# AhmedKishki/AMP-SPARC-SpatialModulation

Hardware: AMD Instinct MI355X
Metric: detected symbol-vectors/sec, VAMP Nt=256 Nr=512 16-QAM; SER match vs ref (higher is better)
Workload: dtype bf16x3; 1 GPU; cfg4: VAMP Nt=256 Nr=512 Na=8 16QAM batch=4096 iterations<=20 EbN0=8.0 dB, one channel per batch; global_batch=4096, parallelism=epoch-shard x1 (independent epochs, one all-reduce of the error counters)

## Files before the change

amp-sparc-spatialmodulation_amd/csrc/amp_persist.h:

```cpp
#pragma once

#include <cfloat>

#include "amp_common.h"

namespace amp {

constexpr int PRING = 4;

typedef float f32x4 __attribute__((ext_vector_type(4)));
typedef unsigned u32x4 __attribute__((ext_vector_type(4)));

__device__ __forceinline__ f32x4 mfma16x16x4(float a, float b, f32x4 c) {
    return __builtin_amdgcn_mfma_f32_16x16x4f32(a, b, c, 0, 0, 0);
}

template <int NT, int G>
__device__ __forceinline__ void gemm16(const float* sA, int lda, const float* __restrict__ wq, int ct0,
                                       f32x4 (&acc)[NT]) {
    constexpr int R = G < PRING ? G : PRING;
    const int lane = threadIdx.x & 63;
#pragma unroll
    for (int t = 0; t < NT; ++t) acc[t] = f32x4{0.f, 0.f, 0.f, 0.f};
    const int ct0u = __builtin_amdgcn_readfirstlane(ct0);
// ... 87 lines not shown
    u32x4 q[6];
#pragma unroll
    for (int h = 0; h < 4; ++h) {
        unsigned a0, a1, a2, b0, b1, b2;
        split3x2(re[2 * h], re[2 * h + 1], a0, a1, a2);
        split3x2(im[2 * h], im[2 * h + 1], b0, b1, b2);
        q[0][h] = a0; q[1][h] = a1; q[2][h] = a2; q[3][h] = b0; q[4][h] = b1; q[5][h] = b2;
    }
    const int c = pl_col(pl_opaque(row), j0, pl_mask(ldx));
#pragma unroll
    for (int f = 0; f < 6; ++f) *reinterpret_cast<u32x4*>(sP + (f * 16 + row) * ldx + c) = q[f];
}

__device__ __forceinline__ float dpp_swap_pair(float v) {
    return __int_as_float(__builtin_amdgcn_update_dpp(0, __float_as_int(v), 0xB1, 0xF, 0xF, false));
}

__device__ __forceinline__ void x3_store_acc(unsigned short* sP, int ldx, int o, const float (&vr)[4],
                                             const float (&vi)[4]) {
    const int lane = pl_opaque((int)threadIdx.x) & 63;
    const bool odd = (lane & 1) != 0;
    float gr[2], gi[2];
#pragma unroll
    for (int h = 0; h < 2; ++h) {
        gr[h] = dpp_swap_pair(odd ? vr[h] : vr[2 + h]);
        gi[h] = dpp_swap_pair(odd ? vi[h] : vi[2 + h]);
    }
    const int row0 = 4 * (lane >> 4) + (odd ? 2 : 0);
    const int m = pl_mask(ldx);
    const int pl = 16 * ldx;
#pragma unroll
    for (int h = 0; h < 2; ++h) {
        unsigned short* p = sP + (row0 + h) * ldx + pl_col(row0 + h, o & ~1, m);
        const float mr = odd ? vr[2 + h] : vr[h], mi = odd ? vi[2 + h] : vi[h];
        unsigned q[6];
        split3x2(odd ? gr[h] : mr, odd ? mr : gr[h], q[0], q[1], q[2]);
        split3x2(odd ? gi[h] : mi, odd ? mi : gi[h], q[3], q[4], q[5]);
#pragma unroll
        for (int f = 0; f < 6; ++f) *reinterpret_cast<unsigned*>(p + f * pl) = q[f];
    }
}

__device__ __forceinline__ void split3(float x, unsigned& p0, unsigned& p1, unsigned& p2) {
    unsigned q0, q1, q2;
    split3x2(x, 0.0f, q0, q1, q2);
    p0 = q0 & 0xffffu; p1 = q1 & 0xffffu; p2 = q2 & 0xffffu;
}

__device__ __forceinline__ bf16x8 as_bf16x8(u32x4 v) { return __builtin_bit_cast(bf16x8, v); }

constexpr int x3_ring_depth(int G, int R) { return G < R ? G : R; }
template <int NT, int RR>
struct X3Ring {
    u32x4 v[RR][NT][6];
};

template <int G>
__device__ __forceinline__ __amdgpu_buffer_rsrc_t x3_wrsrc(const void* wq, int ct0) {
    const int ct0u = __builtin_amdgcn_readfirstlane(ct0);
    return __builtin_amdgcn_make_buffer_rsrc((char*)const_cast<void*>(wq) + (size_t)ct0u * G * 6 * 1024, (short)0,
                                             0x7ffffff0, 0x00020000);
}

template <int NT, int G, int RR, int T0 = 0, int T1 = NT>
__device__ __forceinline__ void x3_ring_load(X3Ring<NT, RR>& ring, int d, __amdgpu_buffer_rsrc_t wr, int g) {
    const int vo = (threadIdx.x & 63) * 16;
#pragma unroll
    for (int t = T0; t < T1; ++t)
#pragma unroll
        for (int f = 0; f < 6; ++f)
            ring.v[d][t][f] = __builtin_amdgcn_raw_buffer_load_b128(wr, vo, ((t * G + g) * 6 + f) * 1024, 0);
}

template <int NT, int G, int R = 1, int T0 = 0, int T1 = NT>
__device__ __forceinline__ void x3_ring_fill(X3Ring<NT, x3_ring_depth(G, R)>& ring, const void* __restrict__ wq, int ct0) {
    const __amdgpu_buffer_rsrc_t wr = x3_wrsrc<G>(wq, ct0);
#pragma unroll
    for (int d = 0; d < x3_ring_depth(G, R); ++d) x3_ring_load<NT, G, x3_ring_depth(G, R), T0, T1>(ring, d, wr, d);
}

struct X3NoHook {
    __device__ __forceinline__ void operator()(int) const {}
};
template <int NT, int G, int R = 1, bool PIN = false, bool HL = false, bool NEXT = false, class Hook = X3NoHook>
__device__ __forceinline__ void gemm_x3_ring(const unsigned short* sP, int ldx, const void* __restrict__ wq, int ct0,
                                             X3Ring<NT, x3_ring_depth(G, R)>& ring, f32x4 (&cr)[NT], f32x4 (&ci)[NT],
                                             const void* __restrict__ wq_next = nullptr, Hook&& hook = Hook()) {
    constexpr int RR = x3_ring_depth(G, R);
    static_assert(!NEXT || G % RR == 0, "the next operator's group j lands in slot j % RR");
    constexpr int NL = HL ? NT : 1;
    const int lane = threadIdx.x & 63;
    f32x4 lr[NL], li[NL];
#pragma unroll
    for (int t = 0; t < NT; ++t) { cr[t] = f32x4{0.f, 0.f, 0.f, 0.f}; ci[t] = f32x4{0.f, 0.f, 0.f, 0.f}; }
#pragma unroll
    for (int t = 0; t < NL; ++t) { lr[t] = f32x4{0.f, 0.f, 0.f, 0.f}; li[t] = f32x4{0.f, 0.f, 0.f, 0.f}; }
    const __amdgpu_buffer_rsrc_t wr = x3_wrsrc<G>(wq, ct0);
    const int ln = pl_opaque(lane);
    const int sw = (ln & 15) & pl_mask(ldx);
    const unsigned short* ap = sP + (ln & 15) * ldx + 8 * ((ln >> 4) ^ (sw & 3));
    const int s32 = 32 * (sw >> 2);
    const u32x4 sgn = {0x80008000u, 0x80008000u, 0x80008000u, 0x80008000u};
    u32x4 an[6];
    if constexpr (!PIN) {
#pragma unroll
        for (int f = 0; f < 6; ++f) an[f] = *reinterpret_cast<const u32x4*>(ap + s32 + f * 16 * ldx);
    }
#pragma unroll
    for (int g = 0; g < G; ++g) {
        const int d = g % RR;
        u32x4 a[6], na[3];
        if constexpr (PIN) {
#pragma unroll
            for (int f = 0; f < 6; ++f) a[f] = *reinterpret_cast<const u32x4*>(ap + ((32 * g) ^ s32) + f * 16 * ldx);
        } else {
#pragma unroll
            for (int f = 0; f < 6; ++f) a[f] = an[f];
            if (g + 1 < G) {
#pragma unroll
                for (int f = 0; f < 6; ++f)
                    an[f] = *reinterpret_cast<const u32x4*>(ap + ((32 * (g + 1)) ^ s32) + f * 16 * ldx);
            }
        }
#pragma unroll
        for (int f = 0; f < 3; ++f) na[f] = a[3 + f] ^ sgn;
#pragma unroll
        for (int t = 0; t < NT; ++t) {
            const u32x4* w = ring.v[d][t];
            f32x4 gr = cr[t], gi = ci[t];
            f32x4 sr = HL ? lr[HL ? t : 0] : gr, si = HL ? li[HL ? t : 0] : gi;
#define AMP_MF(acc, x, y) acc = __builtin_amdgcn_mfma_f32_16x16x32_bf16(as_bf16x8(x), as_bf16x8(y), acc, 0, 0, 0)
            AMP_MF(sr, a[0], w[2]);  AMP_MF(si, a[0], w[5]);
            AMP_MF(sr, a[1], w[1]);  AMP_MF(si, a[1], w[4]);
            AMP_MF(sr, a[2], w[0]);  AMP_MF(si, a[2], w[3]);
            AMP_MF(sr, na[0], w[5]); AMP_MF(si, a[3], w[2]);
            AMP_MF(sr, na[1], w[4]); AMP_MF(si, a[4], w[1]);
            AMP_MF(sr, na[2], w[3]); AMP_MF(si, a[5], w[0]);
            AMP_MF(sr, a[0], w[1]);  AMP_MF(si, a[0], w[4]);
            AMP_MF(sr, a[1], w[0]);  AMP_MF(si, a[1], w[3]);
            AMP_MF(sr, na[0], w[4]); AMP_MF(si, a[3], w[1]);
            AMP_MF(sr, na[1], w[3]); AMP_MF(si, a[4], w[0]);
            if constexpr (HL) {
                lr[HL ? t : 0] = sr; li[HL ? t : 0] = si;
            } else {
                gr = sr; gi = si;
            }
            AMP_MF(gr, a[0], w[0]);  AMP_MF(gi, a[0], w[3]);
            AMP_MF(gr, na[0], w[3]); AMP_MF(gi, a[3], w[0]);
#undef AMP_MF
            cr[t] = gr; ci[t] = gi;
        }
        if constexpr (PIN) __builtin_amdgcn_sched_barrier(0);
        hook(g);
        if (g + RR < G) {
            x3_ring_load<NT, G>(ring, d, wr, g + RR);
        } else if constexpr (NEXT) {
            x3_ring_load<NT, G>(ring, d, x3_wrsrc<G>(wq_next, ct0), g + RR - G);
        }
        __builtin_amdgcn_sched_barrier(0);
    }
    if constexpr (HL) {
#pragma unroll
        for (int t = 0; t < NT; ++t) { cr[t] += lr[HL ? t : 0]; ci[t] += li[HL ? t : 0]; }
    }
}

template <int NT, int G, int R = 1, bool PIN = false, bool HL = false>
__device__ __forceinline__ void gemm_x3(const unsigned short* sP, int ldx, const void* __restrict__ wq, int ct0,
                                        f32x4 (&cr)[NT], f32x4 (&ci)[NT]) {
    X3Ring<NT, x3_ring_depth(G, R)> ring;
    x3_ring_fill<NT, G, R>(ring, wq, ct0);
    gemm_x3_ring<NT, G, R, PIN, HL>(sP, ldx, wq, ct0, ring, cr, ci);
}

typedef _Float16 f16x8 __attribute__((ext_vector_type(8)));
typedef _Float16 f16x2_t __attribute__((ext_vector_type(2)));
constexpr int H2_EX = 14;
constexpr int YH2_EX = 10;

__device__ __forceinline__ int h2_row_exp(float m) {
    if (!(m > 0.f) || !__builtin_isfinite(m)) return 0;
    return 14 - __builtin_amdgcn_frexp_expf(m);
}

__device__ __forceinline__ void split2x2(float x, float y, unsigned& p0, unsigned& p1) {
    const f32x2_t v = {x, y};
    const f16x2_t h0 = __builtin_convertvector(v, f16x2_t);
    const f32x2_t b = __builtin_convertvector(h0, f32x2_t);
    f32x2_t r = v - b;
    r.x = __builtin_isfinite(b.x) ? r.x : 0.0f;
    r.y = __builtin_isfinite(b.y) ? r.y : 0.0f;
    const f16x2_t h1 = __builtin_convertvector(r, f16x2_t);
    p0 = __builtin_bit_cast(unsigned, h0);
    p1 = __builtin_bit_cast(unsigned, h1);
}

__device__ __forceinline__ void split2(float x, int e, unsigned& p0, unsigned& p1) {
    unsigned q0, q1;
    split2x2(__builtin_amdgcn_ldexpf(x, e), 0.0f, q0, q1);
    p0 = q0 & 0xffffu; p1 = q1 & 0xffffu;
}

__device__ __forceinline__ void h2_store8(unsigned short* sP, int ldx, int row, int j0, const float (&re)[8],
                                          const float (&im)[8]) {
    u32x4 q[4];
#pragma unroll
    for (int h = 0; h < 4; ++h) {
        unsigned a0, a1, b0, b1;
        split2x2(re[2 * h], re[2 * h + 1], a0, a1);
        split2x2(im[2 * h], im[2 * h + 1], b0, b1);
        q[0][h] = a0; q[1][h] = a1; q[2][h] = b0; q[3][h] = b1;
    }
    const int c = pl_col(pl_opaque(row), j0, pl_mask(ldx));
#pragma unroll
    for (int f = 0; f < 4; ++f) *reinterpret_cast<u32x4*>(sP + (f * 16 + row) * ldx + c) = q[f];
}

__device__ __forceinline__ void h2_store_acc(unsigned short* sP, int ldx, int o, const float (&vr)[4],
                                             const float (&vi)[4]) {
    const int lane = pl_opaque((int)threadIdx.x) & 63;
    const bool odd = (lane & 1) != 0;
    float gr[2], gi[2];
#pragma unroll
    for (int h = 0; h < 2; ++h) {
        gr[h] = dpp_swap_pair(odd ? vr[h] : vr[2 + h]);
        gi[h] = dpp_swap_pair(odd ? vi[h] : vi[2 + h]);
    }
    const int row0 = 4 * (lane >> 4) + (odd ? 2 : 0);
    const int m = pl_mask(ldx);
    const int pl = 16 * ldx;
#pragma unroll
    for (int h = 0; h < 2; ++h) {
        unsigned short* p = sP + (row0 + h) * ldx + pl_col(row0 + h, o & ~1, m);
        const float mr = odd ? vr[2 + h] : vr[h], mi = odd ? vi[2 + h] : vi[h];
        unsigned q[4];
        split2x2(odd ? gr[h] : mr, odd ? mr : gr[h], q[0], q[1]);
        split2x2(odd ? gi[h] : mi, odd ? mi : gi[h], q[2], q[3]);
#pragma unroll
        for (int f = 0; f < 4; ++f) *reinterpret_cast<unsigned*>(p + f * pl) = q[f];
    }
}
// ... 346 lines not shown
```

amp-sparc-spatialmodulation_amd/csrc/amp_vamp.h:

```cpp
#pragma once

#include "amp_decide.h"
#include "amp_denoise.h"
#include "amp_gemm.h"
#include "amp_host.h"

namespace amp {

constexpr int RWG = 1024;
constexpr int PBAR_EPOCH = 64;
constexpr int PBAR_WORDS = PBAR_EPOCH + 256;

struct VampK {
    int B, N, n, k, L, M;
    int Bmean;
    int kap0, ncp0, kap1, ncp1, kap2, ncp2, bn2;
    int nblk2, max_iter;
    double noise_var, sparsity;
    const float* Wt0;
    const float* Wt1;
    const float* Wt2;
    const float* s;
    float* s2;
    float* ytil;
    float* w;
    float* r;
    float* xm;
    float* var0;
    float* var1;
    float* secmax;
    float* secabs;
    Partial* parts;
    VampIter* iters;
    amp_status* status;
    int nwg;
    int E, wpe;
    const float* Wq1;
    const float* Wq2;
    Partial* pparts;
    double* pxch;
    unsigned* pbar;
    unsigned gen;
    int ytil_in_kernel;
    const float* Wq0;
    const float* y;
    int dec_on, ibits, Na, Lin;
    const float2* xtrue;
    const long long* sym;
    const long long* idx;
    DecWG* dwg;
    unsigned char* host_rec;
    int fold_in;
    amp_counts* counts;
    unsigned long long* trace;
    int x3;
    const void* Wx1;
    const void* Wx2;
    XState* xs;
    float* dump;
    long long wch;
    int sch;
    int wg_off, nwg_x, row_off;
    float* q0;
    int q0_store, q0_load;
    Const c;
};

struct VampWs {
    float *Wt0, *Wt1, *Wt2, *s2, *ytil, *w, *var1;
    float *secmax, *secabs;
    Partial* parts;
    VampIter* iters;
    float *Wq0, *Wq1, *Wq2;
    float *Wx1, *Wx2;
    Partial* pparts;
    double* pxch;
    unsigned* pbar;
    DecWG* dwg;
    XState* xs;
    float* q0;
    size_t bytes;
};

static void vamp_geometry(const amp_dims* d, int k, VampK& P) {
    P.Na = d->Na; P.Lin = d->Lin;
    P.B = d->B; P.N = d->N; P.n = d->n; P.k = k; P.L = d->L; P.M = d->M;
    P.kap0 = round_up(2 * d->n, GBK); P.ncp0 = round_up(2 * k, 128);
    P.kap1 = round_up(2 * d->N, GBK); P.ncp1 = round_up(2 * k, 128);
    P.bn2 = section_bn(d);
    P.kap2 = round_up(2 * k, GBK); P.ncp2 = round_up(2 * d->N, P.bn2);
    P.nblk2 = cdiv(d->B, GBM) * (P.ncp2 / P.bn2);
}

static VampWs vamp_carve(const amp_dims* d, int k, int max_iter, void* base, int chans = 1) {
    VampK P;
    vamp_geometry(d, k, P);
    Carve cv(base);
    VampWs w;
    w.Wt0 = cv.take<float>((size_t)P.ncp0 * P.kap0);
    w.Wt1 = cv.take<float>((size_t)P.ncp1 * P.kap1);
    w.Wt2 = cv.take<float>((size_t)P.ncp2 * P.kap2);
    w.s2 = cv.take<float>((size_t)k);
    w.ytil = cv.take<float>((size_t)d->B * 2 * k);
    w.w = cv.take<float>((size_t)d->B * 2 * k);
    w.var1 = cv.take<float>((size_t)d->B * d->N);
    w.secmax = cv.take<float>((size_t)d->B * d->L);
    w.secabs = cv.take<float>((size_t)d->B * d->L);
    w.parts = cv.take<Partial>((size_t)max_iter * P.nblk2);
    w.iters = cv.take<VampIter>((size_t)max_iter + 1);
    const int nwg = cdiv(d->B, 16);
    w.Wq0 = cv.take<float>((size_t)2 * k * 2 * d->n * chans);
    w.Wq1 = cv.take<float>((size_t)2 * k * 2 * d->N);
    w.Wq2 = cv.take<float>((size_t)2 * d->N * 2 * k);
    w.Wx1 = cv.take<float>((size_t)3 * k * d->N * chans);
    w.Wx2 = cv.take<float>((size_t)3 * k * d->N * chans);
    w.pxch = cv.take<double>((size_t)max_iter * nwg * 4);
    w.pbar = cv.take<unsigned>(PBAR_WORDS);
    w.pparts = cv.take<Partial>((size_t)max_iter * nwg);
    w.dwg = cv.take<DecWG>((size_t)2 * nwg);
    w.xs = cv.take<XState>(1);
    w.q0 = cv.take<float>((size_t)2 * k);
    w.bytes = cv.off;
    return w;
}

__device__ __forceinline__ float* var_buf(const VampK& P, int t) { return (t & 1) ? P.var1 : P.var0; }

struct S2Lane {
    float v[4];
};
__device__ inline S2Lane s2_lane(const VampK& P, const float* s) {
    S2Lane a;
    const int lane = threadIdx.x & 63;
#pragma unroll
    for (int j = 0; j < 4; ++j) {
        const int i = lane + 64 * j;
        const float x = s[min(i, P.k - 1)];
        a.v[j] = i < P.k ? x * x : 0.f;
    }
    return a;
}

__device__ inline void vamp_lmmse_scalars(const VampK& P, bool first, double s2t64, float s2t, float* lds, VampIter& it,
                                          const S2Lane* sl = nullptr) {
    const float vr = first ? (float)(P.noise_var / s2t64) : (1.0f / s2t) * (float)P.noise_var;
    (void)lds;
    double ss = 0.0;
    if (sl) {
        const int lane = threadIdx.x & 63;
#pragma unroll
        for (int j = 0; j < 4; ++j)
            if (lane + 64 * j < P.k) ss += (double)(1.0f / (sl->v[j] + vr));
    } else {
        for (int i = threadIdx.x & 63; i < P.k; i += 64) ss += (double)(1.0f / (P.s[i] * P.s[i] + vr));
    }
    ss = group_sum(ss, 64);
    const float varL = (float)(ss / (double)P.k) * (float)P.noise_var;
    const double eta = (double)P.k / (double)P.N;
    float xtv, s2t32;
    if (first) {
        xtv = (float)eta * varL + (float)((1.0 - eta) * s2t64);
        s2t32 = (float)s2t64;
    } else {
        xtv = (float)eta * varL + (float)(1.0 - eta) * s2t;
        s2t32 = s2t;
    }
    const float alpha = clampf_t(xtv / s2t32, AMP_VAR_RATIO_MIN, 1.0f - AMP_VAR_RATIO_MIN);
    const float sigma2 = clampf_t((alpha / (1.0f - alpha)) * s2t32, AMP_VAR_MIN, AMP_VAR_MAX);
    it.vr = vr;
    it.alpha = alpha;
    it.inv1ma = 1.0f / (1.0f - alpha);
    it.sigma2 = sigma2;
    it.inv_sigma2 = 1.0f / sigma2;
    it.s2t = s2t32;
}

__device__ inline VampIter vamp_first_iter(const VampK& P, float* lds, const S2Lane* sl = nullptr) {
    VampIter it;
    it.stopped = 0; it.T = 0; it.fixed = 0; it.fixed_all = 0; it.G = 0.0;
    it.pad1[0] = it.pad1[1] = it.pad1[2] = 0.f;
    it.dxdr_prev = 0.f;
    it.ns_prev = 1.f;
    const double p = P.sparsity;
    vamp_lmmse_scalars(P, true, p * p * (1 - p) + (1 - p) * (1 - p) * p, 0.f, lds, it, sl);
    return it;
}

__device__ inline VampIter vamp_advance(const VampK& P, const VampIter& cur, const PartAcc& pa, int fixed, int t,
                                        float* lds, const S2Lane* sl = nullptr) {
    VampIter nx;
    nx.stopped = 0; nx.T = 0; nx.fixed = fixed; nx.fixed_all = (fixed < 0) ? 1 : 0; nx.G = pa.maxabs;
    nx.pad1[0] = nx.pad1[1] = nx.pad1[2] = 0.f;
    if (pa.notclose == 0) {
        nx = cur;
        nx.stopped = 1;
        nx.T = t + 1;
        nx.fixed = fixed;
    } else {
        const float mean = (float)(pa.sumvar / ((double)P.Bmean * (double)P.N));
        const float dxdr = clampf_t(mean / cur.sigma2, AMP_VAR_RATIO_MIN, 1.0f - AMP_VAR_RATIO_MIN);
        const float ns = 1.0f / (1.0f - dxdr);
        const float s2t = clampf_t((cur.sigma2 * dxdr) * ns, AMP_VAR_MIN, AMP_VAR_MAX);
        nx.dxdr_prev = dxdr;
        nx.ns_prev = ns;
        vamp_lmmse_scalars(P, false, 0.0, s2t, lds, nx, sl);
    }
    return nx;
}

__device__ inline amp_status vamp_make_status(const VampK& P, const VampIter& cur, const VampIter& nx, int fixed) {
    amp_status s;
    s.T = nx.stopped ? nx.T : P.max_iter;
    s.nan_state = fixed != 0 ? 1 : 0;
    s.stopped = nx.stopped;
    s.gemm = P.x3 + 1;
    s.last_scalar[0] = cur.s2t; s.last_scalar[1] = cur.alpha; s.last_scalar[2] = cur.sigma2;
    s.last_scalar[3] = nx.stopped ? cur.dxdr_prev : nx.dxdr_prev;
    return s;
}

struct PDenoisePolicy {
    const float* r;
    float* x;
    float* vnew;
    const float* vprev;
    float* sm;
    float* sa;
    int ldr, M, lspr, N;
    float inv;
    __device__ __forceinline__ void load(int sec, int m, float& rr, float& ri, float& it) const {
        const int row = sec >> lspr, sj = sec & ((1 << lspr) - 1);
        const float2 v = *reinterpret_cast<const float2*>(r + row * ldr + 2 * (sj * M + m));
        rr = v.x; ri = v.y; it = inv;
    }
    __device__ __forceinline__ void store(int sec, int m, float xr, float xi, float var, PartAcc& pa) const {
        const int row = sec >> lspr, sj = sec & ((1 << lspr) - 1);
        *reinterpret_cast<float2*>(x + row * ldr + 2 * (sj * M + m)) = make_float2(xr, xi);
        const int vo = row * N + sj * M + m;
        vnew[vo] = var;
        pa.sumvar += (double)var;
        pa.notclose += torch_close(var, vprev[vo]) ? 0u : 1u;
    }
    __device__ __forceinline__ void section(int sec, float smax, float sabs) const {
        sm[sec] = smax;
        sa[sec] = sabs;
    }
    __device__ __forceinline__ void load_r(int sec, int m, float& rr, float& ri) const {
        const int row = sec >> lspr, sj = sec & ((1 << lspr) - 1);
        const float2 v = *reinterpret_cast<const float2*>(r + row * ldr + 2 * (sj * M + m));
        rr = v.x; ri = v.y;
    }
    __device__ __forceinline__ float load_prev(int sec, int m) const {
        const int row = sec >> lspr, sj = sec & ((1 << lspr) - 1);
        return vprev[row * N + sj * M + m];
    }
    __device__ __forceinline__ void store_xv(int sec, int m, float xr, float xi, float var) const {
        const int row = sec >> lspr, sj = sec & ((1 << lspr) - 1);
        *reinterpret_cast<float2*>(x + row * ldr + 2 * (sj * M + m)) = make_float2(xr, xi);
        vnew[row * N + sj * M + m] = var;
    }
    __device__ __forceinline__ void account(float var, float vp, PartAcc& pa) const {
        pa.sumvar += (double)var;
        pa.notclose += torch_close(var, vp) ? 0u : 1u;
    }
    float* dbg = nullptr;
};
__device__ __forceinline__ void den_debug(const PDenoisePolicy& p, int sec, int m, float ze, float vs) {
    if (p.dbg) {
        const int row = sec >> p.lspr, sj = sec & ((1 << p.lspr) - 1);
        p.dbg[row * 2 * p.N + sj * p.M + m] = ze;
        p.dbg[row * 2 * p.N + p.N + sj * p.M + m] = vs;
    }
}

constexpr int PBM = 16;

bool vamp_persist_eligible(const amp_dims* d, int k, int ncu, int epochs = 1, int gemm = AMP_GEMM_AUTO);
int vamp_persist_max_epochs(const amp_dims* d, int k, int ncu, int gemm = AMP_GEMM_AUTO);
int vamp_persist_wg_per_cu(const amp_dims* d, int k, int gemm);
int vamp_gemm_select(const amp_dims* d, int k, int gemm);
bool vamp_persist_x3_fits(int N, int k, int L);
bool vamp_persist_ytil_in_kernel(const VampK& P);
bool vamp_persist_ytil_h2(const VampK& P);
int vamp_persist_launch(const VampK& P, const Const64& c64, const DecConst& dc, hipStream_t st, int ncu);
int device_cu_count();
float* debug_dump_ptr();
bool gemm_f32_requested();
bool persist_wg2();

}
```

amp-sparc-spatialmodulation_amd/csrc/amp_vamp_persist_kernel.h:

```cpp
#pragma once

#include <stdlib.h>

#include <type_traits>

#include "amp_decide_fused.h"
#include "amp_persist.h"
#include "amp_vamp.h"

namespace amp {

constexpr int AMP_TRACE_STRIDE = 10;
#ifndef AMP_OCC2_PK
#define AMP_OCC2_PK 0
#endif
#ifndef AMP_KK4_DU
#define AMP_KK4_DU 4
#endif
#ifndef AMP_X3_W8_PIN
#define AMP_X3_W8_PIN 0
#endif
#ifndef AMP_X3_W8_RING
#define AMP_X3_W8_RING 1
#endif
#ifndef AMP_X3_W8_PKGRID
#define AMP_X3_W8_PKGRID 1
#endif
#ifndef AMP_X3_W8_DENFAST
#define AMP_X3_W8_DENFAST 1
#endif
#ifndef AMP_DECIDE_NARROW
#define AMP_DECIDE_NARROW 1
#endif
#ifndef AMP_X3_DU
#define AMP_X3_DU 2
#endif

struct PLayout {
    int lda, ldr;
    int offA, offR, offX, offV0, offV1, offSM, offSA, offScr, total;
};

__host__ __device__ inline int x3_ldx(int N) { return pl_ldx(N); }
__host__ __device__ inline int x3_plane_floats(int N) { return 6 * 16 * x3_ldx(N) / 2; }

__host__ __device__ inline PLayout playout(int N, int k, int L, bool x3 = false) {
    PLayout y;
    y.lda = (2 * N > 2 * k ? 2 * N : 2 * k) + 4;
    y.ldr = 2 * N + (x3 ? 8 : 4);
    int o = 0;
    y.offA = o; o += (x3 && x3_plane_floats(N) > PBM * y.lda) ? x3_plane_floats(N) : PBM * y.lda;
    y.offR = o; o += PBM * y.ldr;
    y.offX = o; o += PBM * y.ldr;
    y.offV0 = o; o += PBM * N;
    y.offV1 = o; o += PBM * N;
    y.offSM = o; o += PBM * L;
    y.offSA = o; o += PBM * L;
    o = (o + 3) & ~3;
    y.offScr = o; o += 1024;
    y.total = o;
    return y;
}

constexpr int KARG_DC_OFF = karg_second_offset<VampK, DecConst>();

template <int NT, int KK, int NWV, int DU, bool X3, int OCC = 1, bool H2 = false, bool I8 = false>
__global__ __launch_bounds__(64 * NWV, OCC * NWV / 4) void vamp_persist(VampK P_arg, DecConst dc_arg) {
    (void)P_arg;
    (void)dc_arg;
    unsigned long long kbase = karg_base();
    const VampK* Pp = karg_at<VampK>(kbase, 0);
    const DecConst* Dp = karg_at<DecConst>(kbase, KARG_DC_OFF);
#define P (*Pp)
#define dc (*Dp)
    static_assert(!X3 || ((NWV == 4 || (NWV == 8 && !H2 && OCC == 1)) && NT % 2 == 0),
                  "X3: four waves (eight for the bf16x3 two-waves-per-SIMD form), whole complex tiles");
    static_assert(!(H2 && I8) && (!I8 || X3), "I8: a split-precision form of its own");
    constexpr int PKDEN = ((OCC * NWV / 4 == 1) || AMP_OCC2_PK) ? PK_ALL
                          : (NWV == 8 && KK == 16 && AMP_X3_W8_PKGRID) ? PK_GRID : PK_NONE;
    constexpr bool DENFAST = NWV == 8 && OCC == 1 && PKDEN == PK_GRID && AMP_X3_W8_DENFAST;
    constexpr int PWG = 64 * NWV;
    constexpr int NC = X3 ? NT / 2 : 1;
    constexpr int G3 = NT * NWV / 4;
    constexpr int X3R = (NWV == 8) ? AMP_X3_W8_RING : 1;
    constexpr bool X3PIN = NWV == 8 && AMP_X3_W8_PIN;
    constexpr bool X3PF = X3 && !H2 && !I8;
    constexpr int PFT = (NC + 1) / 2;
#define c64 (static_cast<const Const64&>(*Dp))
    extern __shared__ __attribute__((aligned(16))) float lds[];
    __shared__ int s_flag;
    __shared__ double s_d[PWG / 64][4];
    __shared__ float s_hmax[PWG / 64][PBM];
    __shared__ int s_hexp[PBM];
    const PLayout Y = playout(P.N, P.k, P.L, X3);
    float* sA = lds + Y.offA;
    float* sR = lds + Y.offR;
    float* sX = lds + Y.offX;
    float* sM = lds + Y.offSM;
    float* sS = lds + Y.offSA;
    float* scr = lds + Y.offScr;
    const int tid = threadIdx.x, lane = tid & 63, wave = tid >> 6;
    const int wg = blockIdx.x, nwg = gridDim.x;
    const int wgx = wg + P.wg_off, nwx = P.nwg_x;
    const int ep = wgx / P.wpe, wl = wgx - ep * P.wpe, wg0 = ep * P.wpe;
    const int lrow0 = wl * PBM;
    const int row0 = ep * P.B + lrow0 - P.row_off, nrows = min(PBM, P.B - lrow0);
#define ebar (P.pbar + (P.E > 1 ? PBAR_EPOCH + ep : 0))
    const int N = P.N, twoN = 2 * N, twok = 2 * P.k, M = P.M, spr = N / M;
    const float* const sv_ep = P.s + (size_t)ep * P.sch;
#define Wx1 ((const void*)((const char*)P.Wx1 + ep * P.wch))
#define Wx2 ((const void*)((const char*)P.Wx2 + ep * P.wch))
    const int ldr = Y.ldr, lda = Y.lda;
    const int ct0 = wave * NT;
    const int cc0 = wave * NC;
    unsigned short* sP = reinterpret_cast<unsigned short*>(sA);
    const int ldx = x3_ldx(N);
    signed char* sB = reinterpret_cast<signed char*>(sA);
    const int ldb = i8_ldb(N);

    float yt[NT][4], s2c[NT];
#pragma unroll
    for (int t = 0; t < NT; ++t) {
        const int col = X3 ? 2 * (16 * (cc0 + (t < NC ? t : 0)) + (lane & 15)) : 16 * (ct0 + t) + (lane & 15);
        const float sv = sv_ep[col >> 1];
        s2c[t] = sv * sv;
    }
    if (H2 && P.ytil_in_kernel) {
      if constexpr (H2) {
        constexpr int IPY = NT / 2;
        const int n = P.n, ldy = pl_ldx(n);
        const int row = tid % PBM;
        float re[IPY][8], im[IPY][8];
        float m = 0.f;
#pragma unroll
        for (int i = 0; i < IPY; ++i) {
            const int e = tid + i * PWG;
            const int j0 = 8 * (e / PBM);
#pragma unroll
            for (int h = 0; h < 4; ++h) {
                float4 v = *reinterpret_cast<const float4*>(P.y + (size_t)(row0 + max(min(row, nrows - 1), 0)) * 2 * n + 2 * j0 + 4 * h);
                if (!(row < nrows)) v = make_float4(0.f, 0.f, 0.f, 0.f);
                re[i][2 * h] = v.x; im[i][2 * h] = v.y; re[i][2 * h + 1] = v.z; im[i][2 * h + 1] = v.w;
            }
#pragma unroll
            for (int h = 0; h < 8; ++h) m = fmaxf(m, fmaxf(fabsf(re[i][h]), fabsf(im[i][h])));
        }
        m = fmaxf(m, __shfl_xor(m, 16));
        m = fmaxf(m, __shfl_xor(m, 32));
        if (lane < PBM) s_hmax[wave][lane] = m;
        __syncthreads();
        float mr = s_hmax[0][row];
#pragma unroll
        for (int w = 1; w < PWG / 64; ++w) mr = fmaxf(mr, s_hmax[w][row]);
        const int ex = h2_row_exp(mr);
        if (tid < PBM) s_hexp[tid] = ex;
#pragma unroll
        for (int i = 0; i < IPY; ++i) {
            const int e = tid + i * PWG;
#pragma unroll
            for (int h = 0; h < 8; ++h) {
                re[i][h] = __builtin_amdgcn_ldexpf(re[i][h], ex);
                im[i][h] = __builtin_amdgcn_ldexpf(im[i][h], ex);
            }
            h2_store8(sP, ldy, row, 8 * (e / PBM), re[i], im[i]);
        }
        __syncthreads();
        f32x4 yr[NC], yi[NC];
        gemm_h2<NC, 2 * G3>(sP, ldy, P.Wq0, cc0, yr, yi);
#pragma unroll
        for (int r = 0; r < 4; ++r) {
            const float sc = __builtin_amdgcn_ldexpf(1.0f, -(s_hexp[4 * (lane >> 4) + r] + YH2_EX));
#pragma unroll
            for (int t = 0; t < NC; ++t) {
                yt[2 * t][r] = yr[t][r] * sc;
                yt[2 * t + 1][r] = yi[t][r] * sc;
            }
        }
        __syncthreads();
      }
    } else if (X3) {
      if constexpr (!I8) {
#pragma unroll
        for (int t = 0; t < NC; ++t) {
            const int o = 16 * (cc0 + t) + (lane & 15);
#pragma unroll
            for (int r = 0; r < 4; ++r) {
                const int row = 4 * (lane >> 4) + r;
                const bool in = row < nrows;
                const size_t yo = (size_t)(row0 + max(min(row, nrows - 1), 0)) * twok + 2 * o;
                const float a = P.ytil[yo], b = P.ytil[yo + 1];
                yt[2 * t][r] = in ? a : 0.f;
                yt[2 * t + 1][r] = in ? b : 0.f;
            }
        }
      }
    } else if (P.ytil_in_kernel) {
        const int ldy = 4 * N + 4;
        for (int e = tid; e < PBM * N; e += PWG) {
            const int row = e / N, c4 = 4 * (e - row * N);
            float4 v = *reinterpret_cast<const float4*>(P.y + (size_t)(row0 + max(min(row, nrows - 1), 0)) * 4 * N + c4);
            if (!(row < nrows)) v = make_float4(0.f, 0.f, 0.f, 0.f);
            *reinterpret_cast<float4*>(lds + row * ldy + c4) = v;
        }
        __syncthreads();
        f32x4 acc[NT];
        gemm16<NT, 2 * NT * NWV>(lds, ldy, P.Wq0, ct0, acc);
#pragma unroll
        for (int t = 0; t < NT; ++t)
#pragma unroll
            for (int r = 0; r < 4; ++r) yt[t][r] = acc[t][r];
        __syncthreads();
    } else {
#pragma unroll
        for (int t = 0; t < NT; ++t) {
            const int col = 16 * (ct0 + t) + (lane & 15);
#pragma unroll
            for (int r = 0; r < 4; ++r) {
                const int row = 4 * (lane >> 4) + r;
                const float yv = P.ytil[(size_t)(row0 + max(min(row, nrows - 1), 0)) * twok + col];
                yt[t][r] = (row < nrows) ? yv : 0.f;
            }
        }
    }
    VampIter cur;
    {
        const S2Lane s2l = s2_lane(P, sv_ep);
        cur = vamp_first_iter(P, scr, &s2l);
    }
    {
        const float p = (float)P.sparsity;
        for (int e = tid; e < PBM * twoN; e += PWG) {
            const int row = e / twoN, col = e - row * twoN;
            sR[row * ldr + col] = 0.f;
            sX[row * ldr + col] = (row < nrows && (col & 1) == 0) ? p : 0.f;
        }
        for (int e = tid; e < PBM * N; e += PWG) lds[Y.offV1 + e] = 1.0f;
    }

    unsigned long long* trc = P.trace;
    auto stamp = [&](int t, int ph) {
        if (trc && tid == 0 && t < P.max_iter) trc[((size_t)wg * P.max_iter + t) * AMP_TRACE_STRIDE + ph] = __builtin_amdgcn_s_memtime();
    };
    if (trc && tid == 0) {
        trc[(size_t)nwg * P.max_iter * AMP_TRACE_STRIDE + 2 * wg] = __builtin_amdgcn_s_memtime();
        trc[(size_t)nwg * P.max_iter * AMP_TRACE_STRIDE + 2 * wg + 1] = __builtin_amdgcn_s_memrealtime();
    }
    unsigned nbar = 0;
#define grs (gran_rsrc(P.pparts, (unsigned)(P.max_iter * nwx) * 32u))
    int fixed = 0, last_t = 0, aborted = 0;
    VampIter nx = cur;
    auto exchange = [&](int te, float* vnew, const float* vprev) -> bool {
            PartAcc g;
            const S2Lane s2x = s2_lane(P, P.s + (size_t)ep * P.sch);
            const unsigned tag = P.gen * (unsigned)(P.max_iter + 1) + (unsigned)te + 1u;
            if (!part_gather(grs, ((unsigned)te * nwx + wg0) * 32u, P.wpe, tag, P.pbar + 1, g, scr, &s_flag)) return false;
            stamp(te, 6);
            fixed = 0;
            if (part_allnan(g)) {
                if (!cur.fixed_all) {
                    const float qn = __int_as_float(0x7fc00000);
                    for (int e = tid; e < nrows * twoN; e += PWG) sX[(e / twoN) * ldr + e % twoN] = qn;
                    for (int e = tid; e < nrows * N; e += PWG) vnew[e] = qn;
                }
                g.sumvar = __longlong_as_double(0x7ff8000000000000LL);
                g.notclose = 1;
                fixed = -1;
            } else if (part_danger(g)) {
                const double G32 = g.maxabs, slack = logit_slack(G32);
                const float inv = cur.inv_sigma2;
                auto ldf = [=](int s) {
                    const int row = s / spr, sj = s - row * spr;
                    const float* rp = sR + row * ldr + 2 * sj * M;
                    return [=](int m, float& rr, float& ri, float& it) {
                        rr = rp[2 * m]; ri = rp[2 * m + 1]; it = inv;
                    };
                };
                double gm = 0.0;
                for (int s = tid; s < nrows * spr; s += PWG)
                    if ((double)sS[s] >= G32 - slack) gm = fmax(gm, section_absmax_f64(ldf(s), M, c64));
                gm = group_max(gm, 64);
                if (lane == 0) s_d[wave][0] = gm;
                __syncthreads();
                if (tid == 0) {
                    double m4 = 0.0;
                    for (int w = 0; w < PWG / 64; ++w) m4 = fmax(m4, s_d[w][0]);
                    P.pxch[((size_t)te * nwx + wgx) * 4 + 0] = m4;
                }
                if (!grid_sync_on(ebar, P.pbar + 1, ++nbar * (unsigned)P.wpe, &s_flag)) return false;
                double G = 0.0;
                for (int w = wg0; w < wg0 + P.wpe; ++w) G = fmax(G, P.pxch[((size_t)te * nwx + w) * 4 + 0]);
                double dsum = 0.0;
                int dnc = 0, cnt = 0;
                for (int s = tid; s < nrows * spr; s += PWG) {
                    if (!((double)sM[s] - G < AMP_DANGER + slack)) continue;
                    ++cnt;
                    const int row = s / spr, sj = s - row * spr;
                    float* xp = sX + row * ldr + 2 * sj * M;
                    const int v0 = row * N + sj * M;
                    auto st = [&](int m, float xr, float xi, float var) {
                        const float old = vnew[v0 + m];
                        dsum += (double)var - (double)old;
                        dnc += (torch_close(var, vprev[v0 + m]) ? 0 : 1) - (torch_close(old, vprev[v0 + m]) ? 0 : 1);
                        xp[2 * m] = xr; xp[2 * m + 1] = xi;
                        vnew[v0 + m] = var;
                    };
                    exact_section_f64<true>(ldf(s), st, M, c64, G);
                }
                dsum = group_sum(dsum, 64);
                dnc = group_sum(dnc, 64);
                cnt = group_sum(cnt, 64);
                __syncthreads();
                if (lane == 0) { s_d[wave][1] = dsum; s_d[wave][2] = (double)dnc; s_d[wave][3] = (double)cnt; }
                __syncthreads();
                if (tid == 0) {
                    double a = 0.0, b = 0.0, c = 0.0;
                    for (int w = 0; w < PWG / 64; ++w) { a += s_d[w][1]; b += s_d[w][2]; c += s_d[w][3]; }
                    P.pxch[((size_t)te * nwx + wgx) * 4 + 1] = a;
                    P.pxch[((size_t)te * nwx + wgx) * 4 + 2] = b;
                    P.pxch[((size_t)te * nwx + wgx) * 4 + 3] = c;
                }
                if (!grid_sync_on(ebar, P.pbar + 1, ++nbar * (unsigned)P.wpe, &s_flag)) return false;
                double a = 0.0, b = 0.0, c = 0.0;
                for (int w = wg0; w < wg0 + P.wpe; ++w) {
                    const double* q = P.pxch + ((size_t)te * nwx + w) * 4;
                    a += q[1]; b += q[2]; c += q[3];
                }
                g.sumvar += a;
                g.notclose = (uint32_t)((long long)g.notclose + (long long)b);
                g.maxabs = G;
                fixed = (int)c;
            }
        stamp(te, 9);
        nx = vamp_advance(P, cur, g, fixed, te, scr, &s2x);
        stamp(te, 7);
        return true;
    };

    for (int t = 0; t < P.max_iter; ++t) {
        kbase = karg_launder(kbase);
        Pp = karg_at<VampK>(kbase, 0);
        Dp = karg_at<DecConst>(kbase, KARG_DC_OFF);
        last_t = t;
        stamp(t, 0);
        const float* vprev = lds + ((t & 1) ? Y.offV0 : Y.offV1);
        float* vnew = lds + ((t & 1) ? Y.offV1 : Y.offV0);
        f32x4 acc[NT];
        f32x4 cr[NC], ci[NC];
        X3Ring<NC, x3_ring_depth(G3, X3R)> wring;
        if (__builtin_expect(X3 && !H2 && !I8 && t == 0 && P.q0_load != 0, 0)) {
            stamp(t, 1);
            const int lnq = pl_opaque(lane);
#pragma unroll
            for (int t2 = 0; t2 < NC; ++t2) {
                const float2 q = *reinterpret_cast<const float2*>(P.q0 + 2 * (16 * (cc0 + t2) + (lnq & 15)));
#pragma unroll
                for (int r = 0; r < 4; ++r) {
                    const bool in = 4 * (lnq >> 4) + r < nrows;
                    cr[t2][r] = in ? q.x : 0.f;
                    ci[t2][r] = in ? q.y : 0.f;
                }
            }
            x3_ring_fill<NC, G3, X3R>(wring, Wx2, cc0);
        } else {
        if constexpr (H2 || I8) {
            constexpr int IPT = (NT + 3) / 4;
            const int tdp = I8 ? pl_opaque(tid) : tid;
            const int row = tdp % PBM;
            float re[IPT][8], im[IPT][8];
            float m = 0.f;
#pragma unroll
            for (int i = 0; i < IPT; ++i) {
                const int e = tdp + i * PWG;
                const int j0 = 8 * (e / PBM);
                const bool ok = e < PBM * (N >> 3);
#pragma unroll
                for (int h = 0; h < 4; ++h) {
                    float4 x = make_float4(0.f, 0.f, 0.f, 0.f), q = x;
                    if (ok) {
                        x = *reinterpret_cast<const float4*>(sX + row * ldr + 2 * j0 + 4 * h);
                        q = *reinterpret_cast<const float4*>(sR + row * ldr + 2 * j0 + 4 * h);
                    }
                    re[i][2 * h] = (x.x - cur.dxdr_prev * q.x) * cur.ns_prev;
                    im[i][2 * h] = (x.y - cur.dxdr_prev * q.y) * cur.ns_prev;
                    re[i][2 * h + 1] = (x.z - cur.dxdr_prev * q.z) * cur.ns_prev;
                    im[i][2 * h + 1] = (x.w - cur.dxdr_prev * q.w) * cur.ns_prev;
                }
#pragma unroll
                for (int h = 0; h < 8; ++h) {
                    if constexpr (I8) m = i8_absmax(i8_absmax(m, re[i][h]), im[i][h]);
                    else m = fmaxf(m, fmaxf(fabsf(re[i][h]), fabsf(im[i][h])));
                }
            }
            m = fmaxf(m, __shfl_xor(m, 16));
            m = fmaxf(m, __shfl_xor(m, 32));
            if (lane < PBM) s_hmax[wave][lane] = m;
            __syncthreads();
            float mr = s_hmax[0][row];
#pragma unroll
            for (int w = 1; w < PWG / 64; ++w) mr = fmaxf(mr, s_hmax[w][row]);
            const int ex = I8 ? i8_row_exp(mr) : h2_row_exp(mr);
            if (tid < PBM) s_hexp[tid] = ex;
#pragma unroll
            for (int i = 0; i < IPT; ++i) {
                const int e = tdp + i * PWG;
                if (e < PBM * (N >> 3)) {
                    if constexpr (I8) {
                        i8_store8(sB, ldb, row, 8 * (e / PBM), re[i], im[i], ex);
                    } else {
#pragma unroll
                        for (int h = 0; h < 8; ++h) {
                            re[i][h] = __builtin_amdgcn_ldexpf(re[i][h], ex);
                            im[i][h] = __builtin_amdgcn_ldexpf(im[i][h], ex);
                        }
                        h2_store8(sP, ldx, row, 8 * (e / PBM), re[i], im[i]);
                    }
                }
            }
        } else if constexpr (X3) {
            if constexpr (X3PF) {
                x3_ring_fill<NC, G3, X3R, 0, PFT>(wring, Wx1, cc0);
                __builtin_amdgcn_sched_barrier(0);
            }
            const int tdx = NWV == 8 ? pl_opaque(tid) : tid;
            for (int e = tdx; e < PBM * (N >> 3); e += PWG) {
                const int row = e % PBM, j0 = 8 * (e / PBM);
                float re[8], im[8];
#pragma unroll
                for (int h = 0; h < 4; ++h) {
                    const float4 x = *reinterpret_cast<const float4*>(sX + row * ldr + 2 * j0 + 4 * h);
                    const float4 q = *reinterpret_cast<const float4*>(sR + row * ldr + 2 * j0 + 4 * h);
                    re[2 * h] = (x.x - cur.dxdr_prev * q.x) * cur.ns_prev;
                    im[2 * h] = (x.y - cur.dxdr_prev * q.y) * cur.ns_prev;
                    re[2 * h + 1] = (x.z - cur.dxdr_prev * q.z) * cur.ns_prev;
                    im[2 * h + 1] = (x.w - cur.dxdr_prev * q.w) * cur.ns_prev;
                }
                x3_store8(sP, ldx, row, j0, re, im);
            }
            if constexpr (X3PF) {
                __builtin_amdgcn_sched_barrier(0);
                x3_ring_fill<NC, G3, X3R, PFT, NC>(wring, Wx1, cc0);
            }
        } else
        for (int e = tid; e < PBM * (twoN >> 2); e += PWG) {
            const int row = e / (twoN >> 2), c4 = 4 * (e - row * (twoN >> 2));
            const float4 x = *reinterpret_cast<const float4*>(sX + row * ldr + c4);
            const float4 q = *reinterpret_cast<const float4*>(sR + row * ldr + c4);
            *reinterpret_cast<float4*>(sA + row * lda + c4) =
                make_float4((x.x - cur.dxdr_prev * q.x) * cur.ns_prev, (x.y - cur.dxdr_prev * q.y) * cur.ns_prev,
                            (x.z - cur.dxdr_prev * q.z) * cur.ns_prev, (x.w - cur.dxdr_prev * q.w) * cur.ns_prev);
        }
        __syncthreads();
        stamp(t, 1);
        if constexpr (I8) {
            float rowf[4];
#pragma unroll
            for (int r = 0; r < 4; ++r) rowf[r] = i8_row_factor(s_hexp[4 * (lane >> 4) + r]);
            gemm_i8<NC, G3 / 2>(sB, ldb, Wx1, N, cc0, rowf, cr, ci);
        } else if constexpr (H2)
            gemm_h2<NC, G3>(sP, ldx, Wx1, cc0, cr, ci);
        else if constexpr (X3) {
            gemm_x3_ring<NC, G3, X3R, X3PIN, true, true>(sP, ldx, Wx1, cc0, wring, cr, ci, Wx2);
            if (__builtin_expect(t == 0 && P.q0_store != 0 && wg == 0, 0)) {
                const int lns = pl_opaque(lane);
                if (lns < 16) {
#pragma unroll
                    for (int t2 = 0; t2 < NC; ++t2)
                        *reinterpret_cast<float2*>(P.q0 + 2 * (16 * (cc0 + t2) + lns)) = make_float2(cr[t2][0], ci[t2][0]);
                }
            }
        } else
            gemm16<NT, NT * NWV>(sA, lda, P.Wq1, ct0, acc);
        }
        float hsc[4];
        int hew[4];
        if constexpr (H2 || I8) {
#pragma unroll
            for (int r = 0; r < 4; ++r) hsc[r] = I8 ? 1.0f : __builtin_amdgcn_ldexpf(1.0f, -(s_hexp[4 * (lane >> 4) + r] + H2_EX));
            float mrow[4] = {0.f, 0.f, 0.f, 0.f};
#pragma unroll
            for (int t2 = 0; t2 < NC; ++t2) {
                const float sc = 1.0f / (s2c[t2] + cur.vr);
                float ytr[4], yti[4];
                if constexpr (I8) {
                    const int ln = pl_opaque(lane);
                    const int oo = 16 * (cc0 + t2) + (ln & 15);
#pragma unroll
                    for (int r = 0; r < 4; ++r) {
                        const int row = 4 * (ln >> 4) + r;
                        const float2 u = *reinterpret_cast<const float2*>(P.ytil + (size_t)(row0 + max(min(row, nrows - 1), 0)) * twok + 2 * oo);
                        const float2 v = row < nrows ? u : make_float2(0.f, 0.f);
                        ytr[r] = v.x; yti[r] = v.y;
                    }
                } else {
#pragma unroll
                    for (int r = 0; r < 4; ++r) { ytr[r] = yt[2 * t2][r]; yti[r] = yt[2 * t2 + 1][r]; }
                }
#pragma unroll
                for (int r = 0; r < 4; ++r) {
                    const float qr = I8 ? cr[t2][r] : cr[t2][r] * hsc[r], qi = I8 ? ci[t2][r] : ci[t2][r] * hsc[r];
                    cr[t2][r] = sc * (ytr[r] + cur.vr * qr) - qr;
                    ci[t2][r] = sc * (yti[r] + cur.vr * qi) - qi;
                    if constexpr (I8) mrow[r] = i8_absmax(i8_absmax(mrow[r], cr[t2][r]), ci[t2][r]);
                    else mrow[r] = fmaxf(mrow[r], fmaxf(fabsf(cr[t2][r]), fabsf(ci[t2][r])));
                }
            }
#pragma unroll
            for (int r = 0; r < 4; ++r) {
#pragma unroll
                for (int sh = 1; sh < 16; sh <<= 1) mrow[r] = fmaxf(mrow[r], __shfl_xor(mrow[r], sh));
            }
            if ((lane & 15) == 0) {
#pragma unroll
                for (int r = 0; r < 4; ++r) s_hmax[wave][4 * (lane >> 4) + r] = mrow[r];
            }
        }
        __syncthreads();
        stamp(t, 2);
        if constexpr (H2 || I8) {
#pragma unroll
            for (int r = 0; r < 4; ++r) {
                float mr = s_hmax[0][4 * (lane >> 4) + r];
#pragma unroll
                for (int w = 1; w < PWG / 64; ++w) mr = fmaxf(mr, s_hmax[w][4 * (lane >> 4) + r]);
                hew[r] = I8 ? i8_row_exp(mr) : h2_row_exp(mr);
            }
            const int lnw = I8 ? pl_opaque(lane) : lane;
#pragma unroll
            for (int t2 = 0; t2 < NC; ++t2) {
                const int o = 16 * (cc0 + t2) + (lnw & 15);
                if constexpr (I8) {
                    int wr[4], wi[4];
#pragma unroll
                    for (int r = 0; r < 4; ++r) { wr[r] = i8_fix(cr[t2][r], hew[r]); wi[r] = i8_fix(ci[t2][r], hew[r]); }
                    i8_store_acc(sB, ldb, o, wr, wi);
                } else {
                    float wr[4], wi[4];
#pragma unroll
                    for (int r = 0; r < 4; ++r) {
                        wr[r] = __builtin_amdgcn_ldexpf(cr[t2][r], hew[r]);
                        wi[r] = __builtin_amdgcn_ldexpf(ci[t2][r], hew[r]);
                    }
                    h2_store_acc(sP, ldx, o, wr, wi);
                }
// ... 216 lines not shown
```

Before: 6.021 million symbol-vectors/s.

## Split VAMP advance and overlap scalar tail with first GEMM group

Splits the per-iteration VAMP state update into a head (after the grid exchange) and a tail (LMMSE variance sum, alpha, sigma2). The tail now runs inside the next iteration's x3 ring GEMM, after the first group's loads are issued, so it overlaps with weight streaming instead of sitting on the critical path after the barrier. Singular values are cached in LDS once rather than reloaded from global memory at each exchange. This adds a callback hook to the GEMM loop and relies on cur.sigma2 and the other fields not being consumed before group 0 finishes.

New measurement: 6.104 million symbol-vectors/s (median of 6 runs). 1.4% higher.

```diff
diff --git a/amp-sparc-spatialmodulation_amd/csrc/amp_persist.h b/amp-sparc-spatialmodulation_amd/csrc/amp_persist.h
--- a/amp-sparc-spatialmodulation_amd/csrc/amp_persist.h
+++ b/amp-sparc-spatialmodulation_amd/csrc/amp_persist.h
@@ -193,10 +193,12 @@
 struct X3NoHook {
     __device__ __forceinline__ void operator()(int) const {}
 };
-template <int NT, int G, int R = 1, bool PIN = false, bool HL = false, bool NEXT = false, class Hook = X3NoHook>
+template <int NT, int G, int R = 1, bool PIN = false, bool HL = false, bool NEXT = false, class Hook = X3NoHook,
+          class After = X3NoHook>
 __device__ __forceinline__ void gemm_x3_ring(const unsigned short* sP, int ldx, const void* __restrict__ wq, int ct0,
                                              X3Ring<NT, x3_ring_depth(G, R)>& ring, f32x4 (&cr)[NT], f32x4 (&ci)[NT],
-                                             const void* __restrict__ wq_next = nullptr, Hook&& hook = Hook()) {
+                                             const void* __restrict__ wq_next = nullptr, Hook&& hook = Hook(),
+                                             After&& after = After()) {
     constexpr int RR = x3_ring_depth(G, R);
     static_assert(!NEXT || G % RR == 0, "the next operator's group j lands in slot j % RR");
     constexpr int NL = HL ? NT : 1;
@@ -268,6 +270,7 @@
         } else if constexpr (NEXT) {
             x3_ring_load<NT, G>(ring, d, x3_wrsrc<G>(wq_next, ct0), g + RR - G);
         }
+        after(g);
         __builtin_amdgcn_sched_barrier(0);
     }
     if constexpr (HL) {
diff --git a/amp-sparc-spatialmodulation_amd/csrc/amp_vamp.h b/amp-sparc-spatialmodulation_amd/csrc/amp_vamp.h
--- a/amp-sparc-spatialmodulation_amd/csrc/amp_vamp.h
+++ b/amp-sparc-spatialmodulation_amd/csrc/amp_vamp.h
@@ -35,6 +35,7 @@
     amp_status* status;
     int nwg;
     int E, wpe;
+    float etaf;
     const float* Wq1;
     const float* Wq2;
     Partial* pparts;
@@ -51,6 +52,7 @@
     DecWG* dwg;
     unsigned char* host_rec;
     int fold_in;
+    float ometaf;
     amp_counts* counts;
     unsigned long long* trace;
     int x3;
@@ -85,6 +87,8 @@
 static void vamp_geometry(const amp_dims* d, int k, VampK& P) {
     P.Na = d->Na; P.Lin = d->Lin;
     P.B = d->B; P.N = d->N; P.n = d->n; P.k = k; P.L = d->L; P.M = d->M;
+    const double eta = (double)k / (double)d->N;
+    P.etaf = (float)eta; P.ometaf = (float)(1.0 - eta);
     P.kap0 = round_up(2 * d->n, GBK); P.ncp0 = round_up(2 * k, 128);
     P.kap1 = round_up(2 * d->N, GBK); P.ncp1 = round_up(2 * k, 128);
     P.bn2 = section_bn(d);
@@ -208,6 +212,49 @@
     return nx;
 }
 
+__device__ inline VampIter vamp_advance_head(const VampK& P, const VampIter& cur, const PartAcc& pa, int fixed, int t) {
+    VampIter nx;
+    nx.stopped = 0; nx.T = 0; nx.fixed = fixed; nx.fixed_all = (fixed < 0) ? 1 : 0; nx.G = pa.maxabs;
+    nx.pad1[0] = nx.pad1[1] = nx.pad1[2] = 0.f;
+    nx.vr = nx.alpha = nx.inv1ma = nx.sigma2 = nx.inv_sigma2 = 0.f;
+    if (pa.notclose == 0) {
+        nx = cur;
+        nx.stopped = 1;
+        nx.T = t + 1;
+        nx.fixed = fixed;
+    } else {
+        const float mean = (float)(pa.sumvar / ((double)P.Bmean * (double)P.N));
+        const float dxdr = clampf_t(mean / cur.sigma2, AMP_VAR_RATIO_MIN, 1.0f - AMP_VAR_RATIO_MIN);
+        const float ns = 1.0f / (1.0f - dxdr);
+        nx.dxdr_prev = dxdr;
+        nx.ns_prev = ns;
+        nx.s2t = clampf_t((cur.sigma2 * dxdr) * ns, AMP_VAR_MIN, AMP_VAR_MAX);
+    }
+    return nx;
+}
+
+__device__ inline void vamp_advance_tail(const VampK& P, VampIter& it, const S2Lane& sl) {
+    const float s2t = it.s2t;
+    const float vr = (1.0f / s2t) * (float)P.noise_var;
+    const int lane = threadIdx.x & 63;
+    float q[4];
+#pragma unroll
+    for (int j = 0; j < 4; ++j) q[j] = 1.0f / (sl.v[j] + vr);
+    double ss = 0.0;
+#pragma unroll
+    for (int j = 0; j < 4; ++j) ss += (lane + 64 * j < P.k) ? (double)q[j] : 0.0;
+    ss = group_sum(ss, 64);
+    const float varL = (float)(ss / (double)P.k) * (float)P.noise_var;
+    const float xtv = P.etaf * varL + P.ometaf * s2t;
+    const float alpha = clampf_t(xtv / s2t, AMP_VAR_RATIO_MIN, 1.0f - AMP_VAR_RATIO_MIN);
+    const float sigma2 = clampf_t((alpha / (1.0f - alpha)) * s2t, AMP_VAR_MIN, AMP_VAR_MAX);
+    it.vr = vr;
+    it.alpha = alpha;
+    it.inv1ma = 1.0f / (1.0f - alpha);
+    it.sigma2 = sigma2;
+    it.inv_sigma2 = 1.0f / sigma2;
+}
+
 __device__ inline amp_status vamp_make_status(const VampK& P, const VampIter& cur, const VampIter& nx, int fixed) {
     amp_status s;
     s.T = nx.stopped ? nx.T : P.max_iter;
diff --git a/amp-sparc-spatialmodulation_amd/csrc/amp_vamp_persist_kernel.h b/amp-sparc-spatialmodulation_amd/csrc/amp_vamp_persist_kernel.h
--- a/amp-sparc-spatialmodulation_amd/csrc/amp_vamp_persist_kernel.h
+++ b/amp-sparc-spatialmodulation_amd/csrc/amp_vamp_persist_kernel.h
@@ -34,6 +34,9 @@
 #endif
 #ifndef AMP_X3_DU
 #define AMP_X3_DU 2
+#endif
+#ifndef AMP_SCALAR_TAIL
+#define AMP_SCALAR_TAIL 1
 #endif
 
 struct PLayout {
@@ -86,12 +89,14 @@
     constexpr bool X3PIN = NWV == 8 && AMP_X3_W8_PIN;
     constexpr bool X3PF = X3 && !H2 && !I8;
     constexpr int PFT = (NC + 1) / 2;
+    constexpr int STAIL = (X3PF && OCC == 1) ? AMP_SCALAR_TAIL : 0;
 #define c64 (static_cast<const Const64&>(*Dp))
     extern __shared__ __attribute__((aligned(16))) float lds[];
     __shared__ int s_flag;
     __shared__ double s_d[PWG / 64][4];
     __shared__ float s_hmax[PWG / 64][PBM];
     __shared__ int s_hexp[PBM];
+    __shared__ float s_s2[STAIL != 0 ? 256 : 1];
     const PLayout Y = playout(P.N, P.k, P.L, X3);
     float* sA = lds + Y.offA;
     float* sR = lds + Y.offR;
@@ -226,6 +231,12 @@
     {
         const S2Lane s2l = s2_lane(P, sv_ep);
         cur = vamp_first_iter(P, scr, &s2l);
+        if constexpr (STAIL != 0) {
+            if (wave == 0) {
+#pragma unroll
+                for (int j = 0; j < 4; ++j) s_s2[lane + 64 * j] = s2l.v[j];
+            }
+        }
     }
     {
         const float p = (float)P.sparsity;
@@ -251,7 +262,8 @@
     VampIter nx = cur;
     auto exchange = [&](int te, float* vnew, const float* vprev) -> bool {
             PartAcc g;
-            const S2Lane s2x = s2_lane(P, P.s + (size_t)ep * P.sch);
+            S2Lane s2x;
+            if constexpr (STAIL == 0) s2x = s2_lane(P, P.s + (size_t)ep * P.sch);
             const unsigned tag = P.gen * (unsigned)(P.max_iter + 1) + (unsigned)te + 1u;
             if (!part_gather(grs, ((unsigned)te * nwx + wg0) * 32u, P.wpe, tag, P.pbar + 1, g, scr, &s_flag)) return false;
             stamp(te, 6);
@@ -330,8 +342,12 @@
                 g.maxabs = G;
                 fixed = (int)c;
             }
-        stamp(te, 9);
-        nx = vamp_advance(P, cur, g, fixed, te, scr, &s2x);
+        if constexpr (STAIL != 0) {
+            nx = vamp_advance_head(P, cur, g, fixed, te);
+        } else {
+            stamp(te, 9);
+            nx = vamp_advance(P, cur, g, fixed, te, scr, &s2x);
+        }
         stamp(te, 7);
         return true;
     };
@@ -459,6 +475,18 @@
         } else if constexpr (H2)
             gemm_h2<NC, G3>(sP, ldx, Wx1, cc0, cr, ci);
         else if constexpr (X3) {
+            if constexpr (STAIL != 0) {
+                auto tail0 = [&](int g) __attribute__((always_inline)) {
+                    if (g == 0 && t > 0) {
+                        S2Lane s2x;
+#pragma unroll
+                        for (int j = 0; j < 4; ++j) s2x.v[j] = s_s2[lane + 64 * j];
+                        vamp_advance_tail(P, cur, s2x);
+                        stamp(t, 9);
+                    }
+                };
+                gemm_x3_ring<NC, G3, X3R, X3PIN, true, true>(sP, ldx, Wx1, cc0, wring, cr, ci, Wx2, X3NoHook(), tail0);
+            } else
             gemm_x3_ring<NC, G3, X3R, X3PIN, true, true>(sP, ldx, Wx1, cc0, wring, cr, ci, Wx2);
             if (__builtin_expect(t == 0 && P.q0_store != 0 && wg == 0, 0)) {
                 const int lns = pl_opaque(lane);
```
